# OmicsML/dance

Measured on NVIDIA H100. Metric: cells/sec fwd+bwd scGNN, higher is better.
Workload: dtype f32 (wgmma 3xTF32 split GEMMs, fp32 everything else)

## Files before the change

### dance_b200/csrc/gae_tc.cu

```cuda
#include "tc_common.cuh"

#include <stdlib.h>
#include <string.h>

namespace b2 {
namespace gtc {

using namespace tc;

constexpr int BT = 128;
constexpr int CONSUMERS = 256;
constexpr int THREADS = CONSUMERS + 128;
constexpr int PRODUCER_REGS = 40, CONSUMER_REGS = 232;
constexpr int STAGES = 3;
constexpr int MAX_D = 32;
constexpr uint32_t ZS_BYTES = BT * 128;
constexpr int ZS_PLANES = 2;
constexpr size_t MAX_SMEM = 227 * 1024;

static int64_t padded_n(int32_t n) { return ((int64_t)n + BT - 1) / BT * BT; }
template <int DP> constexpr uint32_t zt_bytes() { return (uint32_t)DP * 4 * 128; }

template <int DP, bool TRI>
struct Tiles {
  static constexpr int JW = TRI ? 64 : BT;
  static constexpr uint32_t JS = JW * 128;
  static constexpr uint32_t JT = zt_bytes<DP>() / (BT / JW);
  static constexpr uint32_t STAGE = ZS_PLANES * JS + 2 * JT;
  static constexpr uint32_t ZIT = TRI ? zt_bytes<DP>() : 0;
  static constexpr uint32_t GT = TRI ? 64 * 64 * 4 : 0;
  static constexpr uint32_t RING = ZS_PLANES * ZS_BYTES + 2 * ZIT + 4 * GT;
  static constexpr size_t SMEM = RING + STAGES * STAGE + 16 * STAGES + 1024;
};
static_assert(Tiles<MAX_D, false>::SMEM <= MAX_SMEM && Tiles<MAX_D, true>::SMEM <= MAX_SMEM, "decoder shared memory");

__host__ __device__ __forceinline__ int zt_pos(int jj) { const int q = jj & 7; return (jj & ~7) | ((q & 1) ? 4 + (q >> 1) : (q >> 1)); }
__host__ __device__ __forceinline__ int gt_pos(int i) { return (i & ~15) | ((i & 7) << 1) | ((i >> 3) & 1); }

__device__ __forceinline__ float tf32_trunc(float x) { return __uint_as_float(__float_as_uint(x) & 0xFFFFE000u); }

template <int DP>
__global__ void __launch_bounds__(256)
gae_split_kernel(const float* __restrict__ z, int64_t ldz, int32_t n, int32_t d, int64_t npad, uint8_t* __restrict__ zs_hi,
                 uint8_t* __restrict__ zs_lo, uint8_t* __restrict__ zt_hi, uint8_t* __restrict__ zt_lo) {
  const int64_t total = npad * DP;
  for (int64_t t = (int64_t)blockIdx.x * blockDim.x + threadIdx.x; t < total; t += (int64_t)gridDim.x * blockDim.x) {
    const int64_t row = t / DP;
    const int k = (int)(t % DP);
    const float v = (row < n && k < d) ? z[row * ldz + k] : 0.f;
    const float h = tf32_trunc(v);
    const float l = v - h;
    const int64_t tile = row / BT;
    const int r = (int)(row % BT);
    const size_t so = (size_t)tile * ZS_BYTES + sw128_offset32((uint32_t)r, (uint32_t)k);
    *reinterpret_cast<float*>(zs_hi + so) = h;
    *reinterpret_cast<float*>(zs_lo + so) = l;
    const int p = zt_pos(r);
    const size_t to = (size_t)tile * zt_bytes<DP>() + (size_t)(p >> 5) * (DP * 128) + sw128_offset32((uint32_t)k, (uint32_t)(p & 31));
    *reinterpret_cast<float*>(zt_hi + to) = h;
    *reinterpret_cast<float*>(zt_lo + to) = l;
  }
}

struct Params {
  const float* z;
  int64_t ldz;
  const uint8_t *zs_hi, *zs_lo, *zt_hi, *zt_lo;
  float* dz;
  double* loss_acc;
  float coef;
  int n, d;
  int row_begin, row_end;
  int sb_begin, nb, sym;
  int n_jt;
};

template <int N>
__device__ __forceinline__ void mma_rs(float (&d)[N / 2], const uint32_t (&a)[4], uint64_t b, uint32_t scale_d) {
  if constexpr (N == 8) wgmma_tf32_rs_n8(d, a, b, scale_d);
  else if constexpr (N == 16) wgmma_tf32_rs_n16(d, a, b, scale_d);
  else if constexpr (N == 32) wgmma_tf32_rs_n32(d, a, b, scale_d);
  else wgmma_tf32_rs_n64(d, a, b, scale_d);
}
template <int N>
__device__ __forceinline__ void mma_ss(float (&d)[N / 2], uint64_t a, uint64_t b, uint32_t scale_d) {
  if constexpr (N == 8) wgmma_tf32_ss_n8(d, a, b, scale_d);
  else if constexpr (N == 16) wgmma_tf32_ss_n16(d, a, b, scale_d);
  else if constexpr (N == 32) wgmma_tf32_ss_n32(d, a, b, scale_d);
  else if constexpr (N == 64) wgmma_tf32_ss_n64(d, a, b, scale_d);
  else wgmma_tf32_ss_n128(d, a, b, scale_d);
}

__device__ __forceinline__ float ex2_approx(float x) { float y; asm("ex2.approx.ftz.f32 %0, %1;" : "=f"(y) : "f"(x)); return y; }
__device__ __forceinline__ float lg2_approx(float x) { float y; asm("lg2.approx.ftz.f32 %0, %1;" : "=f"(y) : "f"(x)); return y; }
__device__ __forceinline__ float rcp_approx(float x) { float y; asm("rcp.approx.ftz.f32 %0, %1;" : "=f"(y) : "f"(x)); return y; }
__device__ __forceinline__ void sts_v2(uint32_t addr, float x, float y) {
  asm volatile("st.shared.v2.f32 [%0], {%1, %2};" ::"r"(addr), "f"(x), "f"(y) : "memory");
}

template <bool MASKED, int V>
__device__ __forceinline__ float sigmoid_softplus(float (&S)[V], float (&L)[V], int jbase, int n, bool live_a, bool live_b) {
  constexpr float LOG2E = 1.4426950408889634f, LN2 = 0.6931471805599453f;
  float relu = 0.f, lg = 0.f, prod = 1.f;
#pragma unroll
  for (int v = 0; v < V; ++v) {
    if ((v & 31) == 31) { lg += lg2_approx(prod); prod = 1.f; }
    const float x = S[v];
    const float e = ex2_approx(-fabsf(x) * LOG2E);
    const float inv = rcp_approx(1.f + e);
    float sg = x >= 0.f ? inv : e * inv;
    if constexpr (MASKED) {
      const int j = jbase + 8 * (v >> 2) + (v & 1);
      const bool ok = j < n && (((v >> 1) & 1) ? live_b : live_a);
      relu += ok ? fmaxf(x, 0.f) : 0.f;
      prod *= ok ? 1.f + e : 1.f;
      sg = ok ? sg : 0.f;
    } else {
      relu += fmaxf(x, 0.f);
      prod *= 1.f + e;
    }
    const float hi = tf32_trunc(sg);
    S[v] = hi;
    L[v] = sg - hi;
  }
  return relu + LN2 * (lg + lg2_approx(prod));
}

template <int DP, bool TRI>
__device__ __forceinline__ void decoder_sweep(const Params& p) {
  using T = Tiles<DP, TRI>;
  constexpr int JW = T::JW;
  extern __shared__ __align__(1024) uint8_t smem_raw[];
  uint8_t* smem = reinterpret_cast<uint8_t*>((reinterpret_cast<uintptr_t>(smem_raw) + 1023) & ~(uintptr_t)1023);
  uint8_t* zi_hi = smem;
  uint8_t* zi_lo = smem + ZS_BYTES;
  uint8_t* zit = smem + ZS_PLANES * ZS_BYTES;
  uint8_t* ring = smem + T::RING;
  constexpr uint32_t ATOM = DP * 128;
  constexpr int NB = DP <= 16 ? 4 : 2;
  constexpr int NBM = DP <= 16 ? 2 : 1;
  const uint32_t full_bar = smem_u32(ring + STAGES * T::STAGE), empty_bar = full_bar + 8 * STAGES;

  int row0, row_end, dz_row0, jt0, jt1;
  if constexpr (TRI) {
    row0 = (int)blockIdx.x * BT; row_end = min(p.n, row0 + BT); dz_row0 = 0;
    const int first = row0 / JW;
    const int per = (p.n_jt - first + (int)gridDim.y - 1) / (int)gridDim.y;
    jt0 = first + (int)blockIdx.y * per; jt1 = min(p.n_jt, jt0 + per);
  } else {
    if (p.sym) {
      const int sb = p.sb_begin + (int)(blockIdx.x >> 1);
      const int blk = (blockIdx.x & 1) ? p.nb - 1 - sb : sb;
      if ((blockIdx.x & 1) && blk == sb) return;
      row0 = blk * BT; row_end = min(p.n, row0 + BT); dz_row0 = 0;
    } else {
      row0 = p.row_begin + (int)blockIdx.x * BT; row_end = min(p.row_end, row0 + BT); dz_row0 = p.row_begin;
    }
    const int per = (p.n_jt + (int)gridDim.y - 1) / (int)gridDim.y;
    jt0 = (int)blockIdx.y * per; jt1 = min(p.n_jt, jt0 + per);
  }
  if (jt0 >= jt1) return;
  const int nt = jt1 - jt0;
  const int diag_end = (row0 + BT) / JW;

  const int tid = threadIdx.x;
  if (tid == 0) {
    for (int s = 0; s < STAGES; ++s) { mbar_init(full_bar + 8 * s, 1); mbar_init(empty_bar + 8 * s, CONSUMERS / 32); }
    fence_barrier_init();
  }
  __syncthreads();

  if (tid >= CONSUMERS) {
    asm volatile("setmaxnreg.dec.sync.aligned.u32 %0;" ::"n"(PRODUCER_REGS));
    if (tid == CONSUMERS) {
      for (int i = 0; i < nt; ++i) {
        const int s = i % STAGES;
        if (i >= STAGES) mbar_wait(empty_bar + 8 * s, (uint32_t)((i / STAGES - 1) & 1));
        const uint32_t fb = full_bar + 8 * s, dst = smem_u32(ring + s * T::STAGE);
        const size_t t = (size_t)(jt0 + i);
        mbar_expect_tx(fb, T::STAGE);
        bulk_load(dst, p.zs_hi + t * T::JS, T::JS, fb);
        bulk_load(dst + T::JS, p.zs_lo + t * T::JS, T::JS, fb);
        if constexpr (TRI) {
          for (uint32_t a = 0; a < T::JT / ATOM; ++a) {
            bulk_load(dst + 2 * T::JS + 2 * a * ATOM, p.zt_hi + t * T::JT + a * ATOM, ATOM, fb);
            bulk_load(dst + 2 * T::JS + (2 * a + 1) * ATOM, p.zt_lo + t * T::JT + a * ATOM, ATOM, fb);
          }
        } else {
          bulk_load(dst + 2 * T::JS, p.zt_hi + t * T::JT, T::JT, fb);
          bulk_load(dst + 2 * T::JS + T::JT, p.zt_lo + t * T::JT, T::JT, fb);
        }
      }
    }
    return;
  }

  asm volatile("setmaxnreg.inc.sync.aligned.u32 %0;" ::"n"(CONSUMER_REGS));
  for (int e = tid; e < BT * DP; e += CONSUMERS) {
    const int r = e / DP, k = e % DP;
    const int row = row0 + r;
    const float v = (row < row_end && k < p.d) ? p.z[(int64_t)row * p.ldz + k] : 0.f;
    const float h = tf32_trunc(v);
    const uint32_t o = sw128_offset32((uint32_t)r, (uint32_t)k);
    *reinterpret_cast<float*>(zi_hi + o) = h;
    *reinterpret_cast<float*>(zi_lo + o) = v - h;
    if constexpr (TRI) {
      const int q = gt_pos(r & 63);
      const uint32_t ot = (uint32_t)(r >> 6) * (4 * ATOM) + (uint32_t)(q >> 5) * (2 * ATOM) + sw128_offset32((uint32_t)k, (uint32_t)(q & 31));
      *reinterpret_cast<float*>(zit + ot) = h;
      *reinterpret_cast<float*>(zit + ot + ATOM) = v - h;
    }
  }
  fence_proxy_async();
  asm volatile("bar.sync 1, %0;" ::"n"(CONSUMERS) : "memory");

  const int wg = TRI ? __shfl_sync(0xffffffffu, tid >> 7, 0) : tid >> 7, warp = (tid >> 5) & 3, lane = tid & 31;
  const int ra = row0 + wg * 64 + warp * 16 + (lane >> 2);
  const bool live_a = ra < row_end, live_b = ra + 8 < row_end;
  const uint32_t ai_hi = smem_u32(zi_hi) + wg * 64 * 128, ai_lo = smem_u32(zi_lo) + wg * 64 * 128;
  const bool full_rows = row0 + BT <= row_end;
  uint8_t* gt_hi = zit + 2 * T::ZIT + wg * 2 * T::GT;
  uint8_t* gt_lo = gt_hi + T::GT;
  const uint32_t bi = smem_u32(zit) + wg * (4 * ATOM);
  const float c2 = 2.f * p.coef;

  float dzb[TRI ? 1 : NB][DP / 2], dzs[DP / 2], dzt[DP / 2];
  float dzm[TRI ? NBM : 1][DP], djm[TRI ? NBM : 1][DP], djs[DP / 2];
#pragma unroll
  for (int v = 0; v < DP / 2; ++v) dzt[v] = 0.f;
  double loss = 0.0;

  constexpr bool OVERLAP = TRI && DP <= 8;
  float S[JW / 2], L[JW / 2];
  auto take_turn = [&]() { asm volatile("bar.sync %0, %1;" ::"r"(2 + wg), "n"(CONSUMERS) : "memory"); };
  auto pass_turn = [&]() { asm volatile("bar.arrive %0, %1;" ::"r"(3 - wg), "n"(CONSUMERS) : "memory"); };

  auto issue_s = [&](int i, float (&S)[JW / 2]) {
    const int s = i % STAGES;
    mbar_wait(full_bar + 8 * s, (uint32_t)((i / STAGES) & 1));
    const uint32_t bs_hi = smem_u32(ring + s * T::STAGE), bs_lo = bs_hi + T::JS;
    wgmma_fence();
#pragma unroll
    for (int kk = 0; kk < DP / 8; ++kk) {
      const uint32_t o = kk * 32;
      mma_ss<JW>(S, wgmma_desc_sw128(ai_lo + o), wgmma_desc_sw128(bs_hi + o), kk > 0);
      mma_ss<JW>(S, wgmma_desc_sw128(ai_hi + o), wgmma_desc_sw128(bs_lo + o), 1);
      mma_ss<JW>(S, wgmma_desc_sw128(ai_hi + o), wgmma_desc_sw128(bs_hi + o), 1);
    }
    wgmma_commit();
  };
  auto issue_dz = [&](int i, float (&S)[JW / 2]) {
    const uint32_t bt_hi = smem_u32(ring + (i % STAGES) * T::STAGE) + 2 * T::JS, bt_lo = bt_hi + T::JT;
    wgmma_fence();
#pragma unroll
    for (int kb = 0; kb < JW / 8; ++kb) {
      const uint32_t ahi[4] = {__float_as_uint(S[4 * kb]), __float_as_uint(S[4 * kb + 2]), __float_as_uint(S[4 * kb + 1]),
                               __float_as_uint(S[4 * kb + 3])};
      const uint32_t alo[4] = {__float_as_uint(L[4 * kb]), __float_as_uint(L[4 * kb + 2]), __float_as_uint(L[4 * kb + 1]),
                               __float_as_uint(L[4 * kb + 3])};
      if constexpr (TRI) {
        const uint32_t o = (uint32_t)(kb >> 2) * (2 * ATOM) + (uint32_t)(kb & 3) * 32;
        mma_rs<DP>(dzs, alo, wgmma_desc_sw128(bt_hi + o), kb > 0);
        mma_rs<2 * DP>(dzm[kb % NBM], ahi, wgmma_desc_sw128(bt_hi + o), kb >= NBM);
      } else {
        const uint32_t o = (uint32_t)(kb >> 2) * ATOM + (uint32_t)(kb & 3) * 32;
        mma_rs<DP>(dzs, alo, wgmma_desc_sw128(bt_hi + o), kb > 0);
        mma_rs<DP>(dzs, ahi, wgmma_desc_sw128(bt_lo + o), 1);
        mma_rs<DP>(dzb[kb % NB], ahi, wgmma_desc_sw128(bt_hi + o), kb >= NB);
      }
    }
    if constexpr (TRI) {
      const uint32_t ag_hi = smem_u32(gt_hi), ag_lo = smem_u32(gt_lo);
#pragma unroll
      for (int kk = 0; kk < 64 / 8; ++kk) {
        const uint32_t oa = (uint32_t)(kk >> 2) * (64 * 128) + (uint32_t)(kk & 3) * 32;
        const uint32_t ob = (uint32_t)(kk >> 2) * (2 * ATOM) + (uint32_t)(kk & 3) * 32;
        mma_ss<DP>(djs, wgmma_desc_sw128(ag_lo + oa), wgmma_desc_sw128(bi + ob), kk > 0);
        mma_ss<2 * DP>(djm[kk % NBM], wgmma_desc_sw128(ag_hi + oa), wgmma_desc_sw128(bi + ob), kk >= NBM);
      }
    }
    wgmma_commit();
  };
  auto dz_fence = [&]() {
    reg_fence(dzs);
    if constexpr (TRI) {
#pragma unroll
      for (int b = 0; b < NBM; ++b) { reg_fence(dzm[b]); reg_fence(djm[b]); }
      reg_fence(djs);
    } else {
#pragma unroll
      for (int b = 0; b < NB; ++b) reg_fence(dzb[b]);
    }
  };
  auto merged = [&](const float (&acc)[TRI ? NBM : 1][DP], const float (&s)[DP / 2], int v) {
    float t = s[v];
#pragma unroll
    for (int b = 0; b < NBM; ++b) t += acc[b][v] + acc[b][v + DP / 2];
    return t;
  };
  auto retire_dz = [&](int i) {
#pragma unroll
    for (int v = 0; v < DP / 2; ++v) {
      if constexpr (TRI) {
        dzt[v] += merged(dzm, dzs, v);
      } else {
        float t = dzs[v];
#pragma unroll
        for (int b = 0; b < NB; ++b) t += dzb[b][v];
        dzt[v] += t;
      }
    }
    if constexpr (TRI) {
      if (jt0 + i >= diag_end) {
        const int ja = (jt0 + i) * JW + warp * 16 + (lane >> 2);
        const bool vec = (p.d & 1) == 0 && (reinterpret_cast<uintptr_t>(p.dz) & 7) == 0;
#pragma unroll
        for (int v = 0; v < DP / 2; v += 2) {
          const int row = ja + 8 * ((v >> 1) & 1);
          const int col = 8 * (v >> 2) + 2 * (lane & 3);
          const float x = merged(djm, djs, v), y = merged(djm, djs, v + 1);
          if (row >= p.n || col >= p.d) continue;
          float* dst = p.dz + (int64_t)row * p.d + col;
          if (vec) {
            atomicAdd(reinterpret_cast<float2*>(dst), make_float2(c2 * x, c2 * y));
          } else {
            atomicAdd(dst, c2 * x);
            if (col + 1 < p.d) atomicAdd(dst + 1, c2 * y);
          }
        }
      }
    }
    __syncwarp();
    if (lane == 0) mbar_arrive(empty_bar + 8 * (i % STAGES));
  };
  auto elementwise = [&](int i, float (&S)[JW / 2]) {
    const int jbase = (jt0 + i) * JW + 2 * (lane & 3);
    const float l = full_rows && (jt0 + i + 1) * JW <= p.n ? sigmoid_softplus<false>(S, L, jbase, p.n, live_a, live_b)
                                                           : sigmoid_softplus<true>(S, L, jbase, p.n, live_a, live_b);
    if constexpr (TRI) {
      loss += (jt0 + i >= diag_end ? 2.0 : 1.0) * (double)l;
      const uint32_t k = (uint32_t)gt_pos(warp * 16 + (lane >> 2));
      const uint32_t base = (k >> 5) * (64 * 128);
#pragma unroll
      for (int c = 0; c < JW / 8; ++c) {
#pragma unroll
        for (int e = 0; e < 2; ++e) {
          const uint32_t o = base + sw128_offset32((uint32_t)(8 * c + 2 * (lane & 3) + e), k & 31);
          sts_v2(smem_u32(gt_hi) + o, S[4 * c + e], S[4 * c + 2 + e]);
          sts_v2(smem_u32(gt_lo) + o, L[4 * c + e], L[4 * c + 2 + e]);
        }
      }
      fence_proxy_async();
    } else {
      loss += (double)l;
    }
  };

  if constexpr (OVERLAP) {
    float S2[JW / 2];
    auto turn = [&](int i, float (&Sp)[JW / 2], float (&Sn)[JW / 2]) {
      take_turn();
      issue_dz(i - 1, Sp);
      issue_s(i, Sn);
      pass_turn();
      wgmma_wait<1>();
      dz_fence();
      retire_dz(i - 1);
      wgmma_wait<0>();
      reg_fence(Sn);
      elementwise(i, Sn);
    };
    auto last = [&](float (&Sp)[JW / 2]) {
      take_turn();
      issue_dz(nt - 1, Sp);
      if (wg == 0) pass_turn();
      wgmma_wait<0>();
      dz_fence();
      retire_dz(nt - 1);
    };
    if (wg == 1) take_turn();
    issue_s(0, S);
    pass_turn();
    wgmma_wait<0>();
    reg_fence(S);
    elementwise(0, S);
    for (int i = 1;; i += 2) {
      if (i == nt) { last(S); break; }
      turn(i, S, S2);
      if (i + 1 == nt) { last(S2); break; }
      turn(i + 1, S2, S);
    }
  } else {
    auto run_dz = [&](int i) {
      issue_dz(i, S);
      wgmma_wait<0>();
      dz_fence();
    };
    auto start_s = [&](int i) {
      issue_s(i, S);
      if constexpr (TRI) pass_turn();
    };
    auto finish_s = [&](int i) {
      wgmma_wait<0>();
      reg_fence(S);
      if constexpr (!TRI) pass_turn();
      elementwise(i, S);
    };
    if (wg == 1) take_turn();
    start_s(0);
    finish_s(0);
    for (int i = 1; i < nt; ++i) {
      take_turn();
      run_dz(i - 1);
      start_s(i);
      retire_dz(i - 1);
      finish_s(i);
    }
    take_turn();
    run_dz(nt - 1);
    retire_dz(nt - 1);
    if (wg == 0) pass_turn();
  }

  const bool atomic = TRI || gridDim.y > 1;
#pragma unroll
  for (int v = 0; v < DP / 2; ++v) {
    const int row = ra + 8 * ((v >> 1) & 1);
    const int col = 8 * (v >> 2) + 2 * (lane & 3) + (v & 1);
    if (row >= row_end || col >= p.d) continue;
    float* dst = p.dz + (int64_t)(row - dz_row0) * p.d + col;
    const float val = c2 * dzt[v];
    if (atomic) atomicAdd(dst, val);
    else *dst += val;
  }
  loss = warp_sum(loss);
  if (lane == 0) atomicAdd(p.loss_acc, loss * (double)p.coef);
}

template <int DP>
__global__ void __launch_bounds__(THREADS, 1)
gae_allpairs_tc_kernel(const __grid_constant__ Params p) {
  decoder_sweep<DP, false>(p);
}

template <int DP>
__global__ void __launch_bounds__(THREADS, 1)
gae_tri_tc_kernel(const __grid_constant__ Params p) {
  decoder_sweep<DP, true>(p);
}

size_t workspace_bytes(int32_t n) { return (size_t)padded_n(n) / BT * (ZS_PLANES * ZS_BYTES + 2 * zt_bytes<MAX_D>()); }

int super_blocks(int32_t n) { return (int)((padded_n(n) / BT + 1) / 2); }

bool eligible(int32_t n, int32_t d, int32_t n_rows, size_t ws_bytes) {
  const int mode = path_mode(B2_PATH_GAE_DECODER);
  if (d < 1 || d > MAX_D || mode == 1 || ws_bytes < workspace_bytes(n)) return false;
  return mode == 2 || (int64_t)n * n_rows >= (1ll << 22);
}

template <int DP, bool TRI>
static int launch_sweep(const Params& p, int units, cudaStream_t st) {
  int splits = tuning(B2_TUNE_GAE_SPLITS);
  if (splits <= 0) splits = ceil_div(sm_count(), units);
  if (splits > p.n_jt) splits = p.n_jt;
  if (splits < 1) splits = 1;
  auto kernel = TRI ? gae_tri_tc_kernel<DP> : gae_allpairs_tc_kernel<DP>;
  constexpr size_t smem = Tiles<DP, TRI>::SMEM;
  static bool attr_set = false;
  if (!attr_set) {
    B2_CHECK_CUDA(cudaFuncSetAttribute(kernel, cudaFuncAttributeMaxDynamicSharedMemorySize, (int)smem));
    attr_set = true;
  }
  kernel<<<dim3((unsigned)units, (unsigned)splits), THREADS, smem, st>>>(p);
  B2_CHECK_LAUNCH(TRI ? "gae_tri_tc_kernel" : "gae_allpairs_tc_kernel");
  return B2_OK;
}

template <int DP>
static int launch_dp(Params p, int units, bool tri, void* ws, cudaStream_t st) {
  const int64_t npad = padded_n(p.n);
  p.nb = (int)(npad / BT);
  uint8_t* zs_hi = reinterpret_cast<uint8_t*>(ws);
  uint8_t* zs_lo = zs_hi + (size_t)p.nb * ZS_BYTES;
  uint8_t* zt_hi = zs_lo + (size_t)p.nb * ZS_BYTES;
  uint8_t* zt_lo = zt_hi + (size_t)p.nb * zt_bytes<DP>();
  int64_t blocks = ceil_div<int64_t>(npad * DP, 256);
  const int64_t cap = (int64_t)sm_count() * 16;
  if (blocks > cap) blocks = cap;
  gae_split_kernel<DP><<<(unsigned)blocks, 256, 0, st>>>(p.z, p.ldz, p.n, p.d, npad, zs_hi, zs_lo, zt_hi, zt_lo);
  B2_CHECK_LAUNCH("gae_split_kernel");
  if (units <= 0) return B2_OK;
  p.zs_hi = zs_hi; p.zs_lo = zs_lo; p.zt_hi = zt_hi; p.zt_lo = zt_lo;
  if (tri) {
    p.n_jt = ceil_div(p.n, Tiles<DP, true>::JW);
    return launch_sweep<DP, true>(p, units, st);
  }
  p.n_jt = p.nb;
  return launch_sweep<DP, false>(p, units, st);
}

int launch(const float* z, int64_t ldz, int32_t n, int32_t d, bool sym, int32_t begin, int32_t end, float coef, float* dz,
           double* loss_acc, void* ws, cudaStream_t st) {
  Params p;
  memset(&p, 0, sizeof(p));
  p.z = z; p.ldz = ldz; p.n = n; p.d = d; p.coef = coef; p.dz = dz; p.loss_acc = loss_acc; p.sym = sym;
  int units;
  if (sym) {
    p.sb_begin = begin;
    units = 2 * (end - begin);
  } else {
    p.row_begin = begin; p.row_end = end;
    units = ceil_div(end - begin, BT);
  }
  const bool tri = !sym && begin == 0 && end == n;
  if (d <= 8) return launch_dp<8>(p, units, tri, ws, st);
  if (d <= 16) return launch_dp<16>(p, units, tri, ws, st);
  return launch_dp<32>(p, units, tri, ws, st);
}

}
}
```

Before: 991,500.

## Offload triangle transpose-gradient GEMM to a dedicated dJ warpgroup

Adds a fourth warpgroup to the triangle decoder kernel. It computes the transposed-side gradient GEMM (G^T·z) and the atomic scatter into dz, handing off G tiles through a pair of full/empty mbarriers. This takes that wgmma and atomic work off the critical path of the two consumer warpgroups, and overlap is now enabled for all DP values. In exchange, registers are rebalanced: consumer and producer budgets shrink to fit the extra warpgroup, and consumers must block on gt_empty before writing G, which risks spills or stalls.

```diff
diff --git a/dance_b200/csrc/gae_tc.cu b/dance_b200/csrc/gae_tc.cu
--- a/dance_b200/csrc/gae_tc.cu
+++ b/dance_b200/csrc/gae_tc.cu
@@ -11,7 +11,14 @@
 constexpr int BT = 128;
 constexpr int CONSUMERS = 256;
 constexpr int THREADS = CONSUMERS + 128;
+constexpr int TRI_THREADS = THREADS + 128;
 constexpr int PRODUCER_REGS = 40, CONSUMER_REGS = 232;
+template <int DP>
+struct TriRegs {
+  static constexpr int PRODUCER = 24, DJ = DP <= 16 ? 80 : 96, CONSUMER = DP <= 16 ? 200 : 192;
+};
+static_assert(128 * (TriRegs<16>::PRODUCER + TriRegs<16>::DJ + 2 * TriRegs<16>::CONSUMER) <= 65536 &&
+              128 * (TriRegs<32>::PRODUCER + TriRegs<32>::DJ + 2 * TriRegs<32>::CONSUMER) <= 65536, "triangle registers");
 constexpr int STAGES = 3;
 constexpr int MAX_D = 32;
 constexpr uint32_t ZS_BYTES = BT * 128;
@@ -30,7 +37,7 @@
   static constexpr uint32_t ZIT = TRI ? zt_bytes<DP>() : 0;
   static constexpr uint32_t GT = TRI ? 64 * 64 * 4 : 0;
   static constexpr uint32_t RING = ZS_PLANES * ZS_BYTES + 2 * ZIT + 4 * GT;
-  static constexpr size_t SMEM = RING + STAGES * STAGE + 16 * STAGES + 1024;
+  static constexpr size_t SMEM = RING + STAGES * STAGE + 16 * STAGES + (TRI ? 32 : 0) + 1024;
 };
 static_assert(Tiles<MAX_D, false>::SMEM <= MAX_SMEM && Tiles<MAX_D, true>::SMEM <= MAX_SMEM, "decoder shared memory");
 
@@ -126,6 +133,14 @@
   return relu + LN2 * (lg + lg2_approx(prod));
 }
 
+template <int NBM, int DP>
+__device__ __forceinline__ float merged(const float (&acc)[NBM][DP], const float (&s)[DP / 2], int v) {
+  float t = s[v];
+#pragma unroll
+  for (int b = 0; b < NBM; ++b) t += acc[b][v] + acc[b][v + DP / 2];
+  return t;
+}
+
 template <int DP, bool TRI>
 __device__ __forceinline__ void decoder_sweep(const Params& p) {
   using T = Tiles<DP, TRI>;
@@ -140,6 +155,7 @@
   constexpr int NB = DP <= 16 ? 4 : 2;
   constexpr int NBM = DP <= 16 ? 2 : 1;
   const uint32_t full_bar = smem_u32(ring + STAGES * T::STAGE), empty_bar = full_bar + 8 * STAGES;
+  const uint32_t gt_full = empty_bar + 8 * STAGES, gt_empty = gt_full + 16;
 
   int row0, row_end, dz_row0, jt0, jt1;
   if constexpr (TRI) {
@@ -162,16 +178,84 @@
   if (jt0 >= jt1) return;
   const int nt = jt1 - jt0;
   const int diag_end = (row0 + BT) / JW;
+  const int handed0 = max(jt0, diag_end) - jt0;
 
   const int tid = threadIdx.x;
   if (tid == 0) {
     for (int s = 0; s < STAGES; ++s) { mbar_init(full_bar + 8 * s, 1); mbar_init(empty_bar + 8 * s, CONSUMERS / 32); }
+    if constexpr (TRI) {
+      for (int w = 0; w < 2; ++w) { mbar_init(gt_full + 8 * w, 4); mbar_init(gt_empty + 8 * w, 4); }
+    }
     fence_barrier_init();
   }
   __syncthreads();
 
+  if constexpr (TRI) {
+    if (tid >= THREADS) {
+      asm volatile("setmaxnreg.dec.sync.aligned.u32 %0;" ::"n"(TriRegs<DP>::DJ));
+      if (handed0 >= nt) return;
+      const int t = tid - THREADS, warp = t >> 5, lane = t & 31;
+      for (int e = t; e < BT * DP; e += 128) {
+        const int r = e / DP, k = e % DP;
+        const int row = row0 + r;
+        const float v = (row < row_end && k < p.d) ? p.z[(int64_t)row * p.ldz + k] : 0.f;
+        const float h = tf32_trunc(v);
+        const int q = gt_pos(r & 63);
+        const uint32_t ot = (uint32_t)(r >> 6) * (4 * ATOM) + (uint32_t)(q >> 5) * (2 * ATOM) + sw128_offset32((uint32_t)k, (uint32_t)(q & 31));
+        *reinterpret_cast<float*>(zit + ot) = h;
+        *reinterpret_cast<float*>(zit + ot + ATOM) = v - h;
+      }
+      fence_proxy_async();
+      asm volatile("bar.sync 4, 128;" ::: "memory");
+      const bool vec = (p.d & 1) == 0 && (reinterpret_cast<uintptr_t>(p.dz) & 7) == 0;
+      const float c2 = 2.f * p.coef;
+      float djm[NBM][DP], djs[DP / 2], djt[DP / 2];
+      for (int i = handed0; i < nt; ++i) {
+        const uint32_t parity = (uint32_t)((i - handed0) & 1);
+#pragma unroll
+        for (int h = 0; h < 2; ++h) {
+          mbar_wait(gt_full + 8 * h, parity);
+          const uint32_t ag_hi = smem_u32(zit + 2 * T::ZIT + h * 2 * T::GT), ag_lo = ag_hi + T::GT;
+          const uint32_t bi = smem_u32(zit) + h * (4 * ATOM);
+          wgmma_fence();
+#pragma unroll
+          for (int kk = 0; kk < 64 / 8; ++kk) {
+            const uint32_t oa = (uint32_t)(kk >> 2) * (64 * 128) + (uint32_t)(kk & 3) * 32;
+            const uint32_t ob = (uint32_t)(kk >> 2) * (2 * ATOM) + (uint32_t)(kk & 3) * 32;
+            mma_ss<DP>(djs, wgmma_desc_sw128(ag_lo + oa), wgmma_desc_sw128(bi + ob), kk > 0);
+            mma_ss<2 * DP>(djm[kk % NBM], wgmma_desc_sw128(ag_hi + oa), wgmma_desc_sw128(bi + ob), kk >= NBM);
+          }
+          wgmma_commit();
+          wgmma_wait<0>();
+          reg_fence(djs);
+#pragma unroll
+          for (int b = 0; b < NBM; ++b) reg_fence(djm[b]);
+          __syncwarp();
+          if (lane == 0) mbar_arrive(gt_empty + 8 * h);
+#pragma unroll
+          for (int v = 0; v < DP / 2; ++v) djt[v] = (h ? djt[v] : 0.f) + merged(djm, djs, v);
+        }
+        const int ja = (jt0 + i) * JW + warp * 16 + (lane >> 2);
+#pragma unroll
+        for (int v = 0; v < DP / 2; v += 2) {
+          const int row = ja + 8 * ((v >> 1) & 1);
+          const int col = 8 * (v >> 2) + 2 * (lane & 3);
+          if (row >= p.n || col >= p.d) continue;
+          float* dst = p.dz + (int64_t)row * p.d + col;
+          if (vec) {
+            atomicAdd(reinterpret_cast<float2*>(dst), make_float2(c2 * djt[v], c2 * djt[v + 1]));
+          } else {
+            atomicAdd(dst, c2 * djt[v]);
+            if (col + 1 < p.d) atomicAdd(dst + 1, c2 * djt[v + 1]);
+          }
+        }
+      }
+      return;
+    }
+  }
+
   if (tid >= CONSUMERS) {
-    asm volatile("setmaxnreg.dec.sync.aligned.u32 %0;" ::"n"(PRODUCER_REGS));
+    asm volatile("setmaxnreg.dec.sync.aligned.u32 %0;" ::"n"(TRI ? TriRegs<DP>::PRODUCER : PRODUCER_REGS));
     if (tid == CONSUMERS) {
       for (int i = 0; i < nt; ++i) {
         const int s = i % STAGES;
@@ -195,7 +279,7 @@
     return;
   }
 
-  asm volatile("setmaxnreg.inc.sync.aligned.u32 %0;" ::"n"(CONSUMER_REGS));
+  asm volatile("setmaxnreg.inc.sync.aligned.u32 %0;" ::"n"(TRI ? TriRegs<DP>::CONSUMER : CONSUMER_REGS));
   for (int e = tid; e < BT * DP; e += CONSUMERS) {
     const int r = e / DP, k = e % DP;
     const int row = row0 + r;
@@ -204,12 +288,6 @@
     const uint32_t o = sw128_offset32((uint32_t)r, (uint32_t)k);
     *reinterpret_cast<float*>(zi_hi + o) = h;
     *reinterpret_cast<float*>(zi_lo + o) = v - h;
-    if constexpr (TRI) {
-      const int q = gt_pos(r & 63);
-      const uint32_t ot = (uint32_t)(r >> 6) * (4 * ATOM) + (uint32_t)(q >> 5) * (2 * ATOM) + sw128_offset32((uint32_t)k, (uint32_t)(q & 31));
-      *reinterpret_cast<float*>(zit + ot) = h;
-      *reinterpret_cast<float*>(zit + ot + ATOM) = v - h;
-    }
   }
   fence_proxy_async();
   asm volatile("bar.sync 1, %0;" ::"n"(CONSUMERS) : "memory");
@@ -221,16 +299,15 @@
   const bool full_rows = row0 + BT <= row_end;
   uint8_t* gt_hi = zit + 2 * T::ZIT + wg * 2 * T::GT;
   uint8_t* gt_lo = gt_hi + T::GT;
-  const uint32_t bi = smem_u32(zit) + wg * (4 * ATOM);
   const float c2 = 2.f * p.coef;
 
   float dzb[TRI ? 1 : NB][DP / 2], dzs[DP / 2], dzt[DP / 2];
-  float dzm[TRI ? NBM : 1][DP], djm[TRI ? NBM : 1][DP], djs[DP / 2];
+  float dzm[TRI ? NBM : 1][DP];
 #pragma unroll
   for (int v = 0; v < DP / 2; ++v) dzt[v] = 0.f;
   double loss = 0.0;
 
-  constexpr bool OVERLAP = TRI && DP <= 8;
+  constexpr bool OVERLAP = TRI;
   float S[JW / 2], L[JW / 2];
   auto take_turn = [&]() { asm volatile("bar.sync %0, %1;" ::"r"(2 + wg), "n"(CONSUMERS) : "memory"); };
   auto pass_turn = [&]() { asm volatile("bar.arrive %0, %1;" ::"r"(3 - wg), "n"(CONSUMERS) : "memory"); };
@@ -269,34 +346,17 @@
         mma_rs<DP>(dzb[kb % NB], ahi, wgmma_desc_sw128(bt_hi + o), kb >= NB);
       }
     }
-    if constexpr (TRI) {
-      const uint32_t ag_hi = smem_u32(gt_hi), ag_lo = smem_u32(gt_lo);
-#pragma unroll
-      for (int kk = 0; kk < 64 / 8; ++kk) {
-        const uint32_t oa = (uint32_t)(kk >> 2) * (64 * 128) + (uint32_t)(kk & 3) * 32;
-        const uint32_t ob = (uint32_t)(kk >> 2) * (2 * ATOM) + (uint32_t)(kk & 3) * 32;
-        mma_ss<DP>(djs, wgmma_desc_sw128(ag_lo + oa), wgmma_desc_sw128(bi + ob), kk > 0);
-        mma_ss<2 * DP>(djm[kk % NBM], wgmma_desc_sw128(ag_hi + oa), wgmma_desc_sw128(bi + ob), kk >= NBM);
-      }
-    }
     wgmma_commit();
   };
   auto dz_fence = [&]() {
     reg_fence(dzs);
     if constexpr (TRI) {
 #pragma unroll
-      for (int b = 0; b < NBM; ++b) { reg_fence(dzm[b]); reg_fence(djm[b]); }
-      reg_fence(djs);
+      for (int b = 0; b < NBM; ++b) reg_fence(dzm[b]);
     } else {
 #pragma unroll
       for (int b = 0; b < NB; ++b) reg_fence(dzb[b]);
     }
-  };
-  auto merged = [&](const float (&acc)[TRI ? NBM : 1][DP], const float (&s)[DP / 2], int v) {
-    float t = s[v];
-#pragma unroll
-    for (int b = 0; b < NBM; ++b) t += acc[b][v] + acc[b][v + DP / 2];
-    return t;
   };
   auto retire_dz = [&](int i) {
 #pragma unroll
@@ -308,26 +368,6 @@
 #pragma unroll
         for (int b = 0; b < NB; ++b) t += dzb[b][v];
         dzt[v] += t;
-      }
-    }
-    if constexpr (TRI) {
-      if (jt0 + i >= diag_end) {
-        const int ja = (jt0 + i) * JW + warp * 16 + (lane >> 2);
-        const bool vec = (p.d & 1) == 0 && (reinterpret_cast<uintptr_t>(p.dz) & 7) == 0;
-#pragma unroll
-        for (int v = 0; v < DP / 2; v += 2) {
-          const int row = ja + 8 * ((v >> 1) & 1);
-          const int col = 8 * (v >> 2) + 2 * (lane & 3);
-          const float x = merged(djm, djs, v), y = merged(djm, djs, v + 1);
-          if (row >= p.n || col >= p.d) continue;
-          float* dst = p.dz + (int64_t)row * p.d + col;
-          if (vec) {
-            atomicAdd(reinterpret_cast<float2*>(dst), make_float2(c2 * x, c2 * y));
-          } else {
-            atomicAdd(dst, c2 * x);
-            if (col + 1 < p.d) atomicAdd(dst + 1, c2 * y);
-          }
-        }
       }
     }
     __syncwarp();
@@ -338,19 +378,26 @@
     const float l = full_rows && (jt0 + i + 1) * JW <= p.n ? sigmoid_softplus<false>(S, L, jbase, p.n, live_a, live_b)
                                                            : sigmoid_softplus<true>(S, L, jbase, p.n, live_a, live_b);
     if constexpr (TRI) {
-      loss += (jt0 + i >= diag_end ? 2.0 : 1.0) * (double)l;
-      const uint32_t k = (uint32_t)gt_pos(warp * 16 + (lane >> 2));
-      const uint32_t base = (k >> 5) * (64 * 128);
-#pragma unroll
-      for (int c = 0; c < JW / 8; ++c) {
-#pragma unroll
-        for (int e = 0; e < 2; ++e) {
-          const uint32_t o = base + sw128_offset32((uint32_t)(8 * c + 2 * (lane & 3) + e), k & 31);
-          sts_v2(smem_u32(gt_hi) + o, S[4 * c + e], S[4 * c + 2 + e]);
-          sts_v2(smem_u32(gt_lo) + o, L[4 * c + e], L[4 * c + 2 + e]);
+      if (i >= handed0) {
+        loss += 2.0 * (double)l;
+        mbar_wait(gt_empty + 8 * wg, (uint32_t)(((i - handed0) & 1) ^ 1));
+        const uint32_t k = (uint32_t)gt_pos(warp * 16 + (lane >> 2));
+        const uint32_t base = (k >> 5) * (64 * 128);
+#pragma unroll
+        for (int c = 0; c < JW / 8; ++c) {
+#pragma unroll
+          for (int e = 0; e < 2; ++e) {
+            const uint32_t o = base + sw128_offset32((uint32_t)(8 * c + 2 * (lane & 3) + e), k & 31);
+            sts_v2(smem_u32(gt_hi) + o, S[4 * c + e], S[4 * c + 2 + e]);
+            sts_v2(smem_u32(gt_lo) + o, L[4 * c + e], L[4 * c + 2 + e]);
+          }
         }
+        fence_proxy_async();
+        __syncwarp();
+        if (lane == 0) mbar_arrive(gt_full + 8 * wg);
+      } else {
+        loss += (double)l;
       }
-      fence_proxy_async();
     } else {
       loss += (double)l;
     }
@@ -396,23 +443,19 @@
       wgmma_wait<0>();
       dz_fence();
     };
-    auto start_s = [&](int i) {
-      issue_s(i, S);
-      if constexpr (TRI) pass_turn();
-    };
     auto finish_s = [&](int i) {
       wgmma_wait<0>();
       reg_fence(S);
-      if constexpr (!TRI) pass_turn();
+      pass_turn();
       elementwise(i, S);
     };
     if (wg == 1) take_turn();
-    start_s(0);
+    issue_s(0, S);
     finish_s(0);
     for (int i = 1; i < nt; ++i) {
       take_turn();
       run_dz(i - 1);
-      start_s(i);
+      issue_s(i, S);
       retire_dz(i - 1);
       finish_s(i);
     }
@@ -444,7 +487,7 @@
 }
 
 template <int DP>
-__global__ void __launch_bounds__(THREADS, 1)
+__global__ void __launch_bounds__(TRI_THREADS, 1)
 gae_tri_tc_kernel(const __grid_constant__ Params p) {
   decoder_sweep<DP, true>(p);
 }
@@ -472,7 +515,7 @@
     B2_CHECK_CUDA(cudaFuncSetAttribute(kernel, cudaFuncAttributeMaxDynamicSharedMemorySize, (int)smem));
     attr_set = true;
   }
-  kernel<<<dim3((unsigned)units, (unsigned)splits), THREADS, smem, st>>>(p);
+  kernel<<<dim3((unsigned)units, (unsigned)splits), TRI ? TRI_THREADS : THREADS, smem, st>>>(p);
   B2_CHECK_LAUNCH(TRI ? "gae_tri_tc_kernel" : "gae_allpairs_tc_kernel");
   return B2_OK;
 }
```

Result: faster. 1.062 million, median of 6 (+7.1%).
